# shayneobrien/generative-models

Measured on NVIDIA H100. Metric: train_step_images_per_sec, higher is better.
Workload: dtype bf16

## Files before the change

generative-models_b200/gm_b200/csrc/engine.cu:

```cuda
#include <cstdarg>
#include <cstdio>
#include <cstring>
#include <map>
#include <string>
#include <vector>

#include "gm_b200.h"
#include "gemm_wgmma.cuh"
#include "kernels.cuh"
#include "conv_ops.cuh"

using namespace gm;

typedef CUresult (*PFN_encodeTiled)(CUtensorMap*, CUtensorMapDataType, cuuint32_t, void*, const cuuint64_t*,
                                    const cuuint64_t*, const cuuint32_t*, const cuuint32_t*, CUtensorMapInterleave,
                                    CUtensorMapSwizzle, CUtensorMapL2promotion, CUtensorMapFloatOOBfill);

struct gm_ctx {
  int device = 0;
  int num_sms = 0;
  PFN_encodeTiled encode = nullptr;
  std::string err;
  long long launches = 0;
  float* scratch = nullptr;
// ... 45 lines not shown
}
static const Sampler kNoSampler = {0u, 1u, 0ull, 0ull, nullptr, 0ull};

static int make_tmap(gm_ctx* c, CUtensorMap* tm, const void* ptr, uint64_t inner, uint64_t outer, uint64_t ld,
                     uint32_t box_inner, uint32_t box_outer, CUtensorMapSwizzle swizzle = CU_TENSOR_MAP_SWIZZLE_128B) {
  if ((reinterpret_cast<uintptr_t>(ptr) & 15) || (ld * 2) % 16 != 0)
    return fail(c, GM_ERR_ARG, "tensor map: pointer/ld must be 16-byte aligned (ptr=%p ld=%llu)", ptr, (unsigned long long)ld);
  cuuint64_t dims[2] = {inner, outer};
  cuuint64_t strides[1] = {ld * 2};
  cuuint32_t box[2] = {box_inner, box_outer};
  cuuint32_t estr[2] = {1, 1};
  CUresult r = c->encode(tm, CU_TENSOR_MAP_DATA_TYPE_BFLOAT16, 2, const_cast<void*>(ptr), dims, strides, box, estr,
                         CU_TENSOR_MAP_INTERLEAVE_NONE, swizzle, CU_TENSOR_MAP_L2_PROMOTION_L2_256B,
                         CU_TENSOR_MAP_FLOAT_OOB_FILL_NONE);
  if (r != CUDA_SUCCESS) return fail(c, GM_ERR_CUDA, "cuTensorMapEncodeTiled failed with %d", int(r));
  return GM_OK;
}

enum PlanKind { PK_NT_208 = 0, PK_NT_64, PK_TN_256, PK_TN_64 };

struct GemmPlan {
  CUtensorMap tmA, tmB;
  CUtensorMap tmA2, tmB2;
  mutable CUtensorMap tmC;
  mutable int tmc_state;
  GemmParams p;
  int kind;
  int grid;
  double flops;
};

static bool g_pdl = true;
static bool g_tma_store = true;
struct ProfAll { const char* name; cudaEvent_t e0, e1; };
static bool g_prof_all = false;
static std::vector<ProfAll> g_prof_all_recs;
template <typename... KArgs, typename... Args>
static cudaError_t launch_pdl(const char* name, void (*kern)(KArgs...), dim3 grid, dim3 block, size_t smem, cudaStream_t s, Args&&... args) {
  struct Scope {
    cudaStream_t s; ProfAll r; bool on;
    Scope(const char* n, cudaStream_t s_) : s(s_), on(g_prof_all) {
      if (on) { r.name = n; cudaEventCreate(&r.e0); cudaEventCreate(&r.e1); cudaEventRecord(r.e0, s); }
    }
    ~Scope() { if (on) { cudaEventRecord(r.e1, s); g_prof_all_recs.push_back(r); } }
  } scope(name, s);
  const bool pdl = g_pdl && strcmp(name, "xhat_kernel") != 0;
  cudaLaunchConfig_t cfg;
  memset(&cfg, 0, sizeof cfg);
  cfg.gridDim = grid;
  cfg.blockDim = block;
  cfg.dynamicSmemBytes = smem;
  cfg.stream = s;
  cudaLaunchAttribute at[1];
  at[0].id = cudaLaunchAttributeProgrammaticStreamSerialization;
  at[0].val.programmaticStreamSerializationAllowed = 1;
  cfg.attrs = at;
  cfg.numAttrs = pdl ? 1 : 0;
  return cudaLaunchKernelEx(&cfg, kern, KArgs(args)...);
}

template <int BN, bool AMN, bool BMN, int EPI = kEpiUniversal, bool SPLIT = false, bool PP = false>
static cudaError_t launch_inst(const GemmPlan& pl, cudaStream_t s) {
  using Cfg = GemmCfg<BN, !AMN, PP>;
  constexpr int CL = kGemmCluster<BN, AMN, BMN>;
  auto kern = gemm_wgmma_kernel<BN, AMN, BMN, EPI, SPLIT, PP>;
  cudaLaunchConfig_t cfg;
  memset(&cfg, 0, sizeof cfg);
  cfg.gridDim = dim3(pl.grid);
  cfg.blockDim = dim3(kGemmThreads);
  cfg.dynamicSmemBytes = Cfg::SMEM_BYTES;
  cfg.stream = s;
  cudaLaunchAttribute at[2];
  int na = 0;
  if (CL > 1) {
    at[na].id = cudaLaunchAttributeClusterDimension;
    at[na].val.clusterDim.x = CL;
    at[na].val.clusterDim.y = 1;
    at[na].val.clusterDim.z = 1;
    ++na;
  }
  static bool configured[64] = {};
  static int max_clusters[64] = {};
  int dev = 0;
  cudaGetDevice(&dev);
  const bool cached = dev >= 0 && dev < 64;
  int mc = cached ? max_clusters[dev] : 0;
  if (!cached || !configured[dev]) {
    cudaError_t e = cudaFuncSetAttribute(kern, cudaFuncAttributeMaxDynamicSharedMemorySize, Cfg::SMEM_BYTES);
    if (e != cudaSuccess) return e;
    if (CL > 1) {
      cfg.gridDim = dim3(CL);
      cfg.attrs = at;
      cfg.numAttrs = na;
      e = cudaOccupancyMaxActiveClusters(&mc, kern, &cfg);
      if (e != cudaSuccess) return e;
      if (mc < 1) return cudaErrorInvalidConfiguration;
    }
    if (cached) { max_clusters[dev] = mc; configured[dev] = true; }
  }
  if (CL > 1) {
    const GemmParams& q = pl.p;
    const int items = cdiv(q.m_tiles, CL) * q.n_tiles * q.splits;
    cfg.gridDim = dim3(CL * (items < mc ? items : mc));
  }
  if (g_pdl) {
    at[na].id = cudaLaunchAttributeProgrammaticStreamSerialization;
    at[na].val.programmaticStreamSerializationAllowed = 1;
    ++na;
  }
  cfg.attrs = at;
  cfg.numAttrs = na;
  GemmParams prm = pl.p;
  prm.tma_store = pl.tmc_state == 1 ? 1 : 0;
  prm.f32_vec = prm.epi == EPI_F32 && !(reinterpret_cast<uintptr_t>(prm.part) & 15) && prm.ldp % 4 == 0 && prm.part_stride % 4 == 0;
  return cudaLaunchKernelEx(&cfg, kern, pl.tmA, pl.tmB, pl.tmC, pl.tmA2, pl.tmB2, prm);
}

template <int BN, bool AMN, bool BMN>
static cudaError_t launch_split(const GemmPlan& pl, cudaStream_t s) {
  return launch_inst<BN, AMN, BMN, kEpiUniversal, true>(pl, s);
}

constexpr int kPingPongMaxKblocks = 7;

static cudaError_t launch_nt208(const GemmPlan& pl, cudaStream_t s) {
  const GemmParams& p = pl.p;
  if (p.epi != EPI_BF16) return launch_inst<208, false, false>(pl, s);
  const bool pp = p.kblocks <= kPingPongMaxKblocks;
#define NT208(S) case S: return launch_inst<208, false, false, S>(pl, s)
#define NT208_PINGPONG(S) case S: return pp ? launch_inst<208, false, false, S, false, true>(pl, s) : launch_inst<208, false, false, S>(pl, s)
  switch (epi_sig(p)) {
    NT208_PINGPONG(epi_sig(ACT_RELU, AUX_NONE, true, DOT_NONE));
    NT208_PINGPONG(epi_sig(ACT_SIGMOID, AUX_NONE, true, DOT_NONE));
    NT208(epi_sig(ACT_RELU, AUX_NONE, true, DOT_W));
    NT208(epi_sig(ACT_RELU, AUX_NONE, true, DOT_W_MASK));
    NT208(epi_sig(ACT_RELU, AUX_NONE, true, DOT_W_PRE));
    NT208(epi_sig(ACT_NONE, AUX_NONE, false, DOT_NONE));
    NT208(epi_sig(ACT_NONE, AUX_NONE, false, DOT_SQ));
// ... 4 lines not shown
    NT208(epi_sig(ACT_SIGMOID, AUX_VAE_OUT, true, DOT_NONE));
    default: return launch_inst<208, false, false>(pl, s);
  }
#undef NT208
#undef NT208_PINGPONG
}

static int launch_plan(gm_ctx* c, const GemmPlan& pl, cudaStream_t s) {
  if (pl.tmc_state == 0) {
    const GemmParams& p = pl.p;
    const bool nt = pl.kind == PK_NT_208 || pl.kind == PK_NT_64;
    pl.tmc_state = 2;
    if (g_tma_store && nt && epi_plain(p.aux_mode, p.dot) && p.nparts == 1 && p.epi == EPI_BF16 && p.out != nullptr && !(reinterpret_cast<uintptr_t>(p.out) & 15) &&
        (p.ldo * 2) % 16 == 0 && p.out_cols > 0) {
      int rc = make_tmap(c, &pl.tmC, p.out, uint64_t(p.out_cols), uint64_t(p.M), uint64_t(p.ldo), kEpiCols, kEpiRows, CU_TENSOR_MAP_SWIZZLE_64B);
      if (rc) return rc;
      pl.tmc_state = 1;
    }
  }
  cudaError_t e;
  gm_ctx::ProfRec rec;
  ProfAll pa;
  if (g_prof_all) {
    static const char* kKind[4] = {"gemm_nt208", "gemm_nt64", "gemm_tn256", "gemm_tn64"};
    static std::map<int, std::string> names;
    const GemmParams& q = pl.p;
    const bool f32 = q.epi == EPI_F32, klong = q.K >= 512, split = q.nparts == 3;
    const int key = epi_sig(q) | (pl.kind | f32 << 2 | klong << 3 | split << 4) << kEpiSigBits;
    auto it = names.find(key);
    if (it == names.end()) {
      char buf[128];
      snprintf(buf, sizeof buf, "%s[act%d aux%d%s%s%s%s%s K%s%s]", kKind[pl.kind], q.act, q.aux_mode, q.bias ? " bias" : "",
               dot_has_w(q.dot) ? " dot" : "", q.dot == DOT_W_PRE ? " pre" : (q.dot == DOT_W_MASK ? " mask" : ""),
               q.dot == DOT_SQ ? " sq" : "", f32 ? " f32" : "", klong ? "long" : "short", split ? " split" : "");
      it = names.emplace(key, buf).first;
    }
    pa.name = it->second.c_str();
    cudaEventCreate(&pa.e0); cudaEventCreate(&pa.e1);
    cudaEventRecord(pa.e0, s);
  }
  if (c->prof) {
    cudaEventCreate(&rec.e0);
    cudaEventCreate(&rec.e1);
    rec.kind = pl.kind;
    rec.flops = pl.flops;
    cudaEventRecord(rec.e0, s);
  }
  if (pl.p.nparts == 3) {
    switch (pl.kind) {
      case PK_NT_208: e = launch_split<208, false, false>(pl, s); break;
      case PK_NT_64: e = launch_split<64, false, false>(pl, s); break;
      case PK_TN_256: e = launch_split<256, true, true>(pl, s); break;
      default: e = launch_split<64, true, true>(pl, s); break;
    }
  } else
  switch (pl.kind) {
    case PK_NT_208: e = launch_nt208(pl, s); break;
    case PK_NT_64: e = launch_inst<64, false, false>(pl, s); break;
    case PK_TN_256: e = launch_inst<256, true, true>(pl, s); break;
    default: e = launch_inst<64, true, true>(pl, s); break;
  }
  c->launches++;
  if (c->prof) {
    cudaEventRecord(rec.e1, s);
    c->prof_recs.push_back(rec);
  }
  if (g_prof_all) { cudaEventRecord(pa.e1, s); g_prof_all_recs.push_back(pa); }
  if (e != cudaSuccess) return fail(c, GM_ERR_CUDA, "GEMM launch failed: %s", cudaGetErrorString(e));
  return GM_OK;
}

static int plan_gemm(gm_ctx* c, GemmPlan* pl, int mode, int M, int N, int K, const void* A, int lda, const void* B,
                     int ldb, int ncover, int max_splits) {
  memset(pl, 0, sizeof *pl);
  if (M <= 0 || N <= 0 || K <= 0) return fail(c, GM_ERR_ARG, "gemm: bad extents %d %d %d", M, N, K);
  int bn, boxn = 0, boxm = BM;
  if (mode == 0) {
    if (ncover <= 64) { pl->kind = PK_NT_64; bn = 64; boxn = 64; }
    else {
      pl->kind = PK_NT_208; bn = 208; boxn = 208 / kGemmCluster<208, false, false>; boxm = kGemmABoxRows<208, false>;
    }
    int rc = make_tmap(c, &pl->tmA, A, K, M, lda, BK, boxm);
    if (rc) return rc;
    rc = make_tmap(c, &pl->tmB, B, K, N, ldb, BK, boxn);
    if (rc) return rc;
  } else {
    if (ncover <= 64) { pl->kind = PK_TN_64; bn = 64; }
    else { pl->kind = PK_TN_256; bn = 256; }
    int rc = make_tmap(c, &pl->tmA, A, M, K, lda, 64, BK);
    if (rc) return rc;
    rc = make_tmap(c, &pl->tmB, B, N, K, ldb, 64, BK);
    if (rc) return rc;
  }
  GemmParams& p = pl->p;
  pl->flops = 2.0 * M * N * K;
  p.M = M; p.N = N; p.K = K;
  p.m_tiles = cdiv(M, BM);
  p.n_tiles = cdiv(ncover, bn);
  p.kblocks = cdiv(K, BK);
  p.nparts = 1; p.kb_part = p.kblocks; p.lo_off = 0;
  pl->tmA2 = pl->tmA; pl->tmB2 = pl->tmB;
  if (c->plan_lo > 0) {
    const __nv_bfloat16* A2 = static_cast<const __nv_bfloat16*>(A) + c->plan_lo;
    const __nv_bfloat16* B2 = static_cast<const __nv_bfloat16*>(B) + c->plan_lo;
    int rc;
    if (mode == 0) {
      if ((rc = make_tmap(c, &pl->tmA2, A2, K, M, lda, BK, boxm))) return rc;
      if ((rc = make_tmap(c, &pl->tmB2, B2, K, N, ldb, BK, boxn))) return rc;
    } else {
      if ((rc = make_tmap(c, &pl->tmA2, A2, M, K, lda, 64, BK))) return rc;
      if ((rc = make_tmap(c, &pl->tmB2, B2, N, K, ldb, 64, BK))) return rc;
    }
    p.nparts = 3; p.kblocks = 3 * p.kb_part; p.lo_off = c->plan_lo;
  }
  const int tiles = p.m_tiles * p.n_tiles;
  const int slots = c->num_sms;
  int splits = 1;
  if (max_splits > 1) {
    splits = slots / tiles;
    if (splits > max_splits) splits = max_splits;
    if (splits > p.kblocks) splits = p.kblocks;
    if (splits < 1) splits = 1;
  }
  p.kb_per_split = cdiv(p.kblocks, splits);
  p.splits = cdiv(p.kblocks, p.kb_per_split);
  const int total = tiles * p.splits;
  pl->grid = total < slots ? total : slots;
  return GM_OK;
}

__global__ void reduce_partials_kernel(const float* __restrict__ part, int nsplit, long long stride, long long rows, int cols,
                                       int ld, float* __restrict__ out) {
  griddep_sync();
  const long long k = blockIdx.x * (long long)blockDim.x + threadIdx.x;
// ... 16 lines not shown
  if (!out) return GM_ERR_ARG;
  *out = nullptr;
  gm_ctx* c = new gm_ctx();
  c->device = device;
  *out = c;
  int n = 0;
  if (cudaGetDeviceCount(&n) != cudaSuccess || n <= 0)
    return fail(c, GM_ERR_CUDA, "no CUDA device visible: this library has no CPU fallback");
  CU_OK(c, cudaSetDevice(device));
  cudaDeviceProp prop;
  CU_OK(c, cudaGetDeviceProperties(&prop, device));
  if (prop.major != 9 || prop.minor != 0)
    return fail(c, GM_ERR_UNSUPPORTED, "device is sm_%d%d; this library is built for sm_90a (H100) only", prop.major, prop.minor);
  c->num_sms = prop.multiProcessorCount;
  void* fn = nullptr;
  cudaDriverEntryPointQueryResult q;
  CU_OK(c, cudaGetDriverEntryPoint("cuTensorMapEncodeTiled", &fn, cudaEnableDefault, &q));
  if (!fn || q != cudaDriverEntryPointSuccess) return fail(c, GM_ERR_CUDA, "cuTensorMapEncodeTiled not available");
  c->encode = reinterpret_cast<PFN_encodeTiled>(fn);
  const char* np = getenv("GM_NO_PDL");
  g_pdl = !(np && np[0] == '1');
  const char* nts = getenv("GM_NO_TMA_STORE");
  g_tma_store = !(nts && nts[0] == '1');
  return GM_OK;
}
extern "C" int gm_ctx_destroy(gm_ctx* c) {
  if (!c) return GM_OK;
  if (c->scratch) cudaFree(c->scratch);
  if (c->red) cudaFree(c->red);
  if (c->loss_zero) cudaFree(c->loss_zero);
  delete c;
  return GM_OK;
}
extern "C" const char* gm_last_error(const gm_ctx* c) { return c ? c->err.c_str() : "null ctx"; }
extern "C" int gm_ctx_num_sms(const gm_ctx* c) { return c ? c->num_sms : 0; }
extern "C" long long gm_launch_count(gm_ctx* c, int reset) {
  if (!c) return 0;
  const long long n = c->launches;
  if (reset) c->launches = 0;
  return n;
}

extern "C" int gm_prof_enable(gm_ctx* c, int on) {
  if (!c) return GM_ERR_ARG;
  c->prof = on == 1;
  g_prof_all = on == 2;
// ... 1208 lines not shown
```

generative-models_b200/gm_b200/csrc/gemm_wgmma.cuh:

```cuda
#pragma once
#include "ptx.cuh"

namespace gm {

constexpr int BM = 128;
constexpr int BK = 64;
constexpr int kMmaK = 16;
constexpr int kProducerThreads = 128;
constexpr int kConsumerWarps = 8;
constexpr int kGemmThreads = kProducerThreads + kConsumerWarps * 32;
constexpr int kBarWg0Issued = 1;
constexpr int kBarWg1Issued = 2;
constexpr int kProducerRegs = 40;
constexpr int kConsumerRegs = 232;
static_assert(kProducerThreads * kProducerRegs + kConsumerWarps * 32 * kConsumerRegs <= 65536, "register file");
constexpr int kSmemBudget = 227 * 1024;

enum : int { EPI_BF16 = 0, EPI_F32 = 1 };
enum : int { ACT_NONE = 0, ACT_RELU = 1, ACT_SIGMOID = 2, ACT_LRELU = 3 };
enum : int { AUX_NONE = 0, AUX_SIGMOID_GRAD = 1, AUX_RELU_MASK = 2, AUX_VAE_OUT = 3, AUX_L1 = 4, AUX_NONZERO_MASK = 5 };
enum : int { DOT_NONE = 0, DOT_W = 1, DOT_SQ = 2, DOT_W_MASK = 3, DOT_W_PRE = 4 };
__host__ __device__ constexpr bool dot_has_w(int dot) { return dot == DOT_W || dot == DOT_W_MASK || dot == DOT_W_PRE; }

constexpr int kEpiUniversal = -1;
// ... 56 lines not shown
struct GemmCfg {
  static constexpr int BN = BN_;
  static constexpr bool PINGPONG = PINGPONG_;
  static_assert(!PINGPONG || (STAGED_EPI && BN == 208), "ping-pong: 128 x 208 K-major kernel only");
  static constexpr int A_ROWS = PINGPONG ? BM / 2 : BM;
  static constexpr int A_BYTES = A_ROWS * BK * 2;
  static constexpr int B_BYTES = BN * BK * 2;
  static constexpr int STAGE_BYTES = A_BYTES + B_BYTES;
  static constexpr int EPI_BYTES = kConsumerWarps * (kEpiScratchBytes + (STAGED_EPI ? kEpiVecBytes : 0));
  static_assert(!STAGED_EPI || (BN + kEpiCols - 1) / kEpiCols <= kEpiVecBlocks, "bias/dot staging too small");
  static constexpr int FIXED_BYTES = 1024 + 512 + EPI_BYTES;
  static constexpr int STAGES_RAW = (kSmemBudget - FIXED_BYTES) / STAGE_BYTES;
  static constexpr int STAGES = STAGES_RAW > 8 ? 8 : STAGES_RAW;
  static constexpr int SMEM_BYTES = STAGES * STAGE_BYTES + FIXED_BYTES;
  static constexpr int BOXN = BN;
  static_assert(BN % 16 == 0 && BN <= 256, "wgmma N constraint (and 16-column epilogue chunks)");
  static_assert(STAGES >= 2, "need a pipeline");
  static_assert(BN < 208 || STAGES >= 4, "the 208- and 256-wide kernels need a 4-stage ring to hide TMA latency");
  static_assert(!PINGPONG || (STAGES == 5 && SMEM_BYTES <= kSmemBudget), "ping-pong ring");
};

template <int BN, bool A_MN, bool B_MN>
constexpr int kGemmCluster = (BN == 208 && !A_MN && !B_MN) ? 2 : 1;

template <int BN, bool A_MN, bool B_MN, int EPI = kEpiUniversal, bool SPLIT = false, bool PINGPONG = false>
__global__ void __launch_bounds__(kGemmThreads, 1)
gemm_wgmma_kernel(const __grid_constant__ CUtensorMap tmA, const __grid_constant__ CUtensorMap tmB,
                  const __grid_constant__ CUtensorMap tmC, const __grid_constant__ CUtensorMap tmA2,
                  const __grid_constant__ CUtensorMap tmB2, const GemmParams p) {
  constexpr bool kUniversal = EPI == kEpiUniversal;
  static_assert(!SPLIT || kUniversal, "split operands: universal epilogue only");
  using Cfg = GemmCfg<BN, !A_MN, PINGPONG>;
  constexpr int STAGES = Cfg::STAGES;
  constexpr int CL = kGemmCluster<BN, A_MN, B_MN>;
  constexpr bool PP = PINGPONG;
  constexpr int A_BOX = kGemmABoxRows<BN, A_MN>;
  static_assert(Cfg::A_ROWS % A_BOX == 0, "A tile in whole boxes");
  static_assert(!B_MN || BN % 64 == 0, "MN-major B needs 64-wide atoms");
  static_assert(CL == 1 || (!B_MN && (BN / CL) % 8 == 0 && (Cfg::B_BYTES / CL) % 1024 == 0), "multicast B share");

  extern __shared__ uint8_t smem_raw[];
  const uint32_t smem_base = (smem_u32(smem_raw) + 1023u) & ~1023u;
  const uint32_t bar_base = smem_base + STAGES * Cfg::STAGE_BYTES;
  auto full_bar = [&](int s) { return bar_base + 8u * s; };
  auto empty_bar = [&](int s) { return bar_base + 8u * (STAGES + s); };
  const uint32_t epi_base = bar_base + 512u;

  const int warp = __shfl_sync(0xffffffffu, int(threadIdx.x >> 5), 0);
  const int lane = threadIdx.x & 31;

  griddep_launch();
  if (warp == 0 && lane == 0) {
    tma_prefetch_desc(&tmA);
    tma_prefetch_desc(&tmB);
    if constexpr (SPLIT) { tma_prefetch_desc(&tmA2); tma_prefetch_desc(&tmB2); }
    if (p.tma_store) tma_prefetch_desc(&tmC);
    for (int s = 0; s < STAGES; ++s) {
      mbar_init(full_bar(s), 1);
      mbar_init(empty_bar(s), CL * (PP ? kConsumerWarps / 2 : kConsumerWarps));
    }
    fence_mbar_init();
  }
  if constexpr (CL > 1) cluster_sync();
  else __syncthreads();
  griddep_wait();

  const int rank = CL > 1 ? int(cluster_ctarank()) : 0;
  const int tiles = (p.m_tiles + CL - 1) / CL * p.n_tiles;
  const int total = tiles * p.splits;
  const int first = blockIdx.x / CL, stride = gridDim.x / CL;
  auto halves_of = [&](int rem) -> int {
    if constexpr (PP) return (rem / p.n_tiles) * CL * BM + Cfg::A_ROWS < p.M ? 2 : 1;
    else return 1;
  };
  auto stage_of = [](uint32_t it) { return int(it % STAGES); };
  auto phase_of = [](uint32_t it) { return (it / STAGES) & 1u; };

  if (warp < kProducerThreads / 32) {
    setmaxnreg_dec<kProducerRegs>();
    if (warp == 0) {
      uint32_t it = 0;
      const bool leader = elect_one();
      for (int item = first; item < total; item += stride) {
        const int split = item / tiles;
        const int rem = item - split * tiles;
        const int m0 = ((rem / p.n_tiles) * CL + rank) * BM;
        const int n0 = (rem % p.n_tiles) * BN;
        const int kb0 = split * p.kb_per_split;
        const int kb1 = min(kb0 + p.kb_per_split, p.kblocks);
        const int nh = halves_of(rem);
        for (int h = 0; h < nh; ++h)
        for (int kb = kb0; kb < kb1; ++kb, ++it) {
          const int stage = stage_of(it);
          mbar_wait(empty_bar(stage), phase_of(it) ^ 1u);
          if (leader) {
            const uint32_t a_dst = smem_base + stage * Cfg::STAGE_BYTES;
            const uint32_t b_dst = a_dst + Cfg::A_BYTES;
            int kk = kb, opart = 0;
            if constexpr (SPLIT) { opart = kb / p.kb_part; kk = kb - opart * p.kb_part; }
            const CUtensorMap* const ta = (SPLIT && opart == 2) ? &tmA2 : &tmA;
            const CUtensorMap* const tb = (SPLIT && opart == 1) ? &tmB2 : &tmB;
            const int k0 = kk * BK;
            mbar_arrive_expect_tx(full_bar(stage), Cfg::STAGE_BYTES);
            if constexpr (!A_MN) {
#pragma unroll
              for (int a = 0; a < Cfg::A_ROWS / A_BOX; ++a)
                tma_load_2d(a_dst + a * (A_BOX * BK * 2), ta, full_bar(stage), k0, m0 + h * Cfg::A_ROWS + a * A_BOX);
            } else {
#pragma unroll
              for (int a = 0; a < BM / 64; ++a)
                tma_load_2d(a_dst + a * (BK * 128), ta, full_bar(stage), m0 + a * 64, k0);
            }
            if constexpr (CL > 1) {
              tma_load_2d_multicast(b_dst + rank * (Cfg::B_BYTES / CL), tb, full_bar(stage), k0, n0 + rank * (BN / CL), (1u << CL) - 1);
            } else if constexpr (!B_MN) {
              tma_load_2d(b_dst, tb, full_bar(stage), k0, n0);
            } else {
#pragma unroll
              for (int b = 0; b < BN / 64; ++b)
                tma_load_2d(b_dst + b * (BK * 128), tb, full_bar(stage), n0 + b * 64, k0);
            }
          }
          __syncwarp();
        }
      }
    }
  } else {
    setmaxnreg_inc<kConsumerRegs>();
    const int cw = warp - kProducerThreads / 32;
    const int wg = cw >> 2;
    const int er = lane & 15;
    const int par = lane >> 4;
    const uint32_t scratch_s = epi_base + uint32_t(cw) * kEpiScratchBytes;
    const uint32_t vec_s = epi_base + kConsumerWarps * kEpiScratchBytes + uint32_t(cw) * kEpiVecBytes;
    const int act = kUniversal ? p.act : epi_act(EPI);
    const int aux_mode = kUniversal ? p.aux_mode : epi_aux(EPI);
    const bool has_bias = kUniversal ? p.bias != nullptr : epi_bias(EPI);
    const int dot_mode = kUniversal ? p.dot : epi_dot(EPI);
    const bool has_dot = dot_has_w(dot_mode);
    const bool store_pre = dot_mode == DOT_W_PRE;
    const bool mask_all = dot_mode == DOT_W_MASK;
    const bool has_sq = dot_mode == DOT_SQ;
    constexpr bool kTmaStore = !A_MN && !SPLIT && (kUniversal ? BN != 208 : epi_plain(epi_aux(EPI), epi_dot(EPI)));
    const bool tma_st = kTmaStore && p.tma_store != 0;
    bool st_pending = false;
    auto stage_acquire = [&]() {
      if (st_pending) {
        if (er == 0) bulk_wait_read();
        __syncwarp();
        st_pending = false;
      }
    };
    constexpr uint32_t A_LBO = A_MN ? BK * 128 : 16, A_KADV = A_MN ? kMmaK * 128 : kMmaK * 2;
    constexpr uint32_t B_LBO = B_MN ? BK * 128 : 16, B_KADV = B_MN ? kMmaK * 128 : kMmaK * 2;
    constexpr uint32_t A_WG_OFF = A_MN ? BK * 128 : 64 * 128;
    constexpr uint32_t DESC_HI = (1024u >> 4) | (1u << 30);
    constexpr int kSteps = (BN + kEpiStep - 1) / kEpiStep;
    float acc[BN / 2];
    auto frag_to_scratch = [&](int s) {
#pragma unroll
      for (int t = 0; t < kSteps; ++t) {
        if (t == s) {
#pragma unroll
          for (int jj = 0; jj < kEpiStep / 8; ++jj) {
            const int j = t * (kEpiStep / 8) + jj;
            if (j < BN / 8) {
#pragma unroll
              for (int h = 0; h < 2; ++h) {
                const int r = (lane >> 2) + 8 * h, c = 8 * jj + 2 * (lane & 3);
                const uint32_t a = scratch_s + uint32_t(r) * (kEpiStep * 4) + ((uint32_t(c >> 2) ^ frag_swz(r)) << 4) + uint32_t(c & 3) * 4;
                asm volatile("st.shared.v2.f32 [%0], {%1, %2};" ::"r"(a), "f"(acc[4 * j + 2 * h]), "f"(acc[4 * j + 2 * h + 1]) : "memory");
              }
            }
          }
        }
      }
    };
    auto scratch_ld16 = [&](int c, uint32_t (&r)[16]) {
#pragma unroll
      for (int i = 0; i < 4; ++i) {
        const uint4 v = lds128(scratch_s + uint32_t(er) * (kEpiStep * 4) + ((uint32_t((c >> 2) + i) ^ frag_swz(er)) << 4));
        r[4 * i] = v.x; r[4 * i + 1] = v.y; r[4 * i + 2] = v.z; r[4 * i + 3] = v.w;
      }
    };
    auto release = [&](int s) {
      __syncwarp();
      if (lane == 0) {
        mbar_arrive(empty_bar(s));
        if constexpr (CL > 1) mbar_arrive_cluster(mapa_shared(empty_bar(s), uint32_t(rank ^ 1)));
      }
    };
    int stage = 0;
    uint32_t phase = 0;
    uint32_t it = 0;
#pragma unroll 1
    for (int item = first; item < total; item += stride) {
      const int split = item / tiles;
      const int rem = item - split * tiles;
      const int n_tile = rem % p.n_tiles;
      const int m0 = ((rem / p.n_tiles) * CL + rank) * BM;
      const int n0 = n_tile * BN;
      const int kb0 = split * p.kb_per_split;
      const int kb1 = min(kb0 + p.kb_per_split, p.kblocks);
      const int nh = halves_of(rem);
      if constexpr (PP) {
        if (wg == 1 || it != 0) named_bar_sync(wg == 1 ? kBarWg0Issued : kBarWg1Issued, kConsumerWarps * 32);
        if (wg == 1 && nh == 1) {
          it += uint32_t(kb1 - kb0);
          if (item + stride < total) named_bar_arrive(kBarWg1Issued, kConsumerWarps * 32);
          continue;
        }
      }
      int prev = -1;
      if constexpr (PP) {
        const uint32_t it0 = it + (wg == 1 ? uint32_t(kb1 - kb0) : 0u);
        stage = stage_of(it0);
        phase = phase_of(it0);
        it += uint32_t(nh * (kb1 - kb0));
      }
#pragma unroll 1
      for (int kb = kb0; kb < kb1; ++kb) {
        mbar_wait(full_bar(stage), phase);
        const uint32_t a_src = smem_base + stage * Cfg::STAGE_BYTES + (PP ? 0u : wg * A_WG_OFF);
        const uint32_t b_src = smem_base + stage * Cfg::STAGE_BYTES + Cfg::A_BYTES;
        const uint32_t a_lo = ((a_src >> 4) & 0x3FFFu) | ((A_LBO >> 4) << 16);
        const uint32_t b_lo = ((b_src >> 4) & 0x3FFFu) | ((B_LBO >> 4) << 16);
        wgmma_pin(acc);
        wgmma_fence();
#pragma unroll
        for (int k = 0; k < BK / kMmaK; ++k) {
          const uint64_t da = (uint64_t(DESC_HI) << 32) | (a_lo + k * (A_KADV >> 4));
          const uint64_t db = (uint64_t(DESC_HI) << 32) | (b_lo + k * (B_KADV >> 4));
          const uint32_t sc = (kb > kb0 || k > 0) ? 1u : 0u;
          if constexpr (BN == 256) wgmma_bf16_n256<A_MN, B_MN>(acc, da, db, sc);
          else if constexpr (BN == 208) wgmma_bf16_n208<A_MN, B_MN>(acc, da, db, sc);
          else wgmma_bf16_n64<A_MN, B_MN>(acc, da, db, sc);
        }
        wgmma_commit();
        wgmma_wait<1>();
        wgmma_pin(acc);
        if (prev >= 0) release(prev);
        prev = stage;
        if (++stage == STAGES) { stage = 0; phase ^= 1u; }
      }
      if constexpr (PP) {
        if (wg == 0 || item + stride < total) named_bar_arrive(wg == 0 ? kBarWg0Issued : kBarWg1Issued, kConsumerWarps * 32);
      }
      wgmma_wait<0>();
      wgmma_pin(acc);
      if (prev >= 0) release(prev);
      const int wrow0 = m0 + wg * 64 + (cw & 3) * 16;
      const int row = wrow0 + er;
      const bool row_ok = row < p.M;
      if (!A_MN && !(kUniversal && p.epi == EPI_F32)) {
        const int lr = lane >> 3, lc = lane & 7;
        constexpr int kBlocks = (BN + kEpiCols - 1) / kEpiCols;
        constexpr bool kAuxAsync = !kUniversal && epi_aux(EPI) != AUX_NONE && epi_dot(EPI) == DOT_NONE && !epi_bias(EPI);
        const uint32_t auxt_s = vec_s;
// ... 21 lines not shown
            const int blk = pass * 4 + (lane >> 3), c4 = (lane & 7) * 4;
            const int c = n0 + blk * kEpiCols + c4;
            uint4 bz = make_uint4(0, 0, 0, 0), wz = bz;
            if (blk < kBlocks && c < p.N) {
              if (has_bias) {
                bz = __ldg(reinterpret_cast<const uint4*>(p.bias + c));
                if (act == ACT_SIGMOID) {
                  bz.x = __float_as_uint(0.5f * __uint_as_float(bz.x)); bz.y = __float_as_uint(0.5f * __uint_as_float(bz.y));
                  bz.z = __float_as_uint(0.5f * __uint_as_float(bz.z)); bz.w = __float_as_uint(0.5f * __uint_as_float(bz.w));
                }
              }
              if (has_dot) wz = __ldg(reinterpret_cast<const uint4*>(p.dot_w + c));
            }
            if (has_bias) sts128(vec_s + (blk * kEpiCols + c4) * 4, bz);
            if (has_dot) sts128(vec_s + kEpiVecBytes / 2 + (blk * kEpiCols + c4) * 4, wz);
          }
          __syncwarp();
        }
        if (aux_mode != AUX_NONE) {
          aux_fetch(0);
          const int nitem = item + stride;
          if (nitem < total) {
            const int nrem = nitem - (nitem / tiles) * tiles;
            const int nm0 = ((nrem / p.n_tiles) * CL + rank) * BM + wg * 64 + (cw & 3) * 16;
            const int nn0 = (nrem % p.n_tiles) * BN;
            for (int t = lane; t < kEpiRows * 4; t += 32) {
              const int r = nm0 + (t >> 2), c = nn0 + (t & 3) * 64;
              if (r < p.M && c < p.out_cols)
                asm volatile("prefetch.global.L2 [%0];" ::"l"(p.aux + size_t(r) * p.ld_aux + c));
            }
          }
        }
        float dot = 0.f;
        float l1_scale = 0.f;
        if (aux_mode == AUX_L1) l1_scale = __ldg(p.row_scale + (row < p.row_split ? 0 : 1));
        if (aux_mode == AUX_SIGMOID_GRAD || aux_mode == AUX_RELU_MASK || aux_mode == AUX_NONZERO_MASK) l1_scale = (p.row_vec != nullptr && row_ok) ? __ldg(p.row_vec + row) : 1.f;
#pragma unroll 1
        for (int s = 0; s < kSteps; ++s) {
          const int cs = s * kEpiStep;
          if (n0 + cs >= p.out_cols) break;
          const int bi = 2 * s + par;
          const int cb = bi * kEpiCols;
          const int col0 = n0 + cb;
          const int nch = (cb >= BN || col0 >= p.out_cols) ? 0 : (BN - cb) >= kEpiCols ? 2 : (BN - cb) / 16;
          const bool last_step = (cs + kEpiStep >= BN) || (n0 + cs + kEpiStep >= p.out_cols);
          const bool step_tma = tma_st && BN - cs >= kEpiStep && wrow0 < p.M;
          stage_acquire();
          frag_to_scratch(s);
// ... 229 lines not shown
```

generative-models_b200/gm_b200/csrc/ptx.cuh:

```cuda
#pragma once
#include <cstdint>
#include <cuda.h>
#include <cuda_bf16.h>
#include <cuda_runtime.h>

namespace gm {

#ifndef GM_WATCHDOG_CYCLES
#define GM_WATCHDOG_CYCLES (4000000000LL)
#endif

__device__ __forceinline__ uint32_t smem_u32(const void* p) {
  return static_cast<uint32_t>(__cvta_generic_to_shared(p));
}

__device__ __forceinline__ bool elect_one() {
  uint32_t pred;
  asm volatile(
      "{\n"
      ".reg .pred p;\n"
      "elect.sync _|p, 0xffffffff;\n"
      "selp.u32 %0, 1, 0, p;\n"
      "}\n"
      : "=r"(pred));
// ... 72 lines not shown
      ::"r"(smem_dst), "l"(reinterpret_cast<uint64_t>(tmap)), "r"(bar), "r"(c0), "r"(c1), "h"(cta_mask)
      : "memory");
}

__device__ __forceinline__ void wgmma_fence() { asm volatile("wgmma.fence.sync.aligned;" ::: "memory"); }
__device__ __forceinline__ void wgmma_commit() { asm volatile("wgmma.commit_group.sync.aligned;" ::: "memory"); }
template <int N>
__device__ __forceinline__ void wgmma_wait() { asm volatile("wgmma.wait_group.sync.aligned %0;" ::"n"(N) : "memory"); }
template <int R>
__device__ __forceinline__ void wgmma_pin(float (&d)[R]) {
#pragma unroll
  for (int i = 0; i < R; ++i) asm volatile("" : "+f"(d[i])::"memory");
}

template <int TA, int TB>
__device__ __forceinline__ void wgmma_bf16_n64(float (&d)[32], uint64_t da, uint64_t db, uint32_t scale_d) {
  asm volatile(
      "{\n"
      ".reg .pred p;\n"
      "setp.ne.b32 p, %34, 0;\n"
      "wgmma.mma_async.sync.aligned.m64n64k16.f32.bf16.bf16 {%0,%1,%2,%3,%4,%5,%6,%7,%8,%9,%10,%11,%12,%13,%14,%15,%16,%17,%18,%19,%20,%21,%22,%23,%24,%25,%26,%27,%28,%29,%30,%31}, %32, %33, p, 1, 1, %35, %36;\n"
      "}\n"
      : "+f"(d[0]), "+f"(d[1]), "+f"(d[2]), "+f"(d[3]), "+f"(d[4]), "+f"(d[5]), "+f"(d[6]), "+f"(d[7]), "+f"(d[8]), "+f"(d[9]), "+f"(d[10]), "+f"(d[11]), "+f"(d[12]), "+f"(d[13]), "+f"(d[14]), "+f"(d[15]), "+f"(d[16]), "+f"(d[17]), "+f"(d[18]), "+f"(d[19]), "+f"(d[20]), "+f"(d[21]), "+f"(d[22]), "+f"(d[23]), "+f"(d[24]), "+f"(d[25]), "+f"(d[26]), "+f"(d[27]), "+f"(d[28]), "+f"(d[29]), "+f"(d[30]), "+f"(d[31])
      : "l"(da), "l"(db), "r"(scale_d), "n"(TA), "n"(TB));
}

template <int TA, int TB>
__device__ __forceinline__ void wgmma_bf16_n208(float (&d)[104], uint64_t da, uint64_t db, uint32_t scale_d) {
  asm volatile(
      "{\n"
      ".reg .pred p;\n"
      "setp.ne.b32 p, %106, 0;\n"
      "wgmma.mma_async.sync.aligned.m64n208k16.f32.bf16.bf16 {%0,%1,%2,%3,%4,%5,%6,%7,%8,%9,%10,%11,%12,%13,%14,%15,%16,%17,%18,%19,%20,%21,%22,%23,%24,%25,%26,%27,%28,%29,%30,%31,%32,%33,%34,%35,%36,%37,%38,%39,%40,%41,%42,%43,%44,%45,%46,%47,%48,%49,%50,%51,%52,%53,%54,%55,%56,%57,%58,%59,%60,%61,%62,%63,%64,%65,%66,%67,%68,%69,%70,%71,%72,%73,%74,%75,%76,%77,%78,%79,%80,%81,%82,%83,%84,%85,%86,%87,%88,%89,%90,%91,%92,%93,%94,%95,%96,%97,%98,%99,%100,%101,%102,%103}, %104, %105, p, 1, 1, %107, %108;\n"
      "}\n"
      : "+f"(d[0]), "+f"(d[1]), "+f"(d[2]), "+f"(d[3]), "+f"(d[4]), "+f"(d[5]), "+f"(d[6]), "+f"(d[7]), "+f"(d[8]), "+f"(d[9]), "+f"(d[10]), "+f"(d[11]), "+f"(d[12]), "+f"(d[13]), "+f"(d[14]), "+f"(d[15]), "+f"(d[16]), "+f"(d[17]), "+f"(d[18]), "+f"(d[19]), "+f"(d[20]), "+f"(d[21]), "+f"(d[22]), "+f"(d[23]), "+f"(d[24]), "+f"(d[25]), "+f"(d[26]), "+f"(d[27]), "+f"(d[28]), "+f"(d[29]), "+f"(d[30]), "+f"(d[31]), "+f"(d[32]), "+f"(d[33]), "+f"(d[34]), "+f"(d[35]), "+f"(d[36]), "+f"(d[37]), "+f"(d[38]), "+f"(d[39]), "+f"(d[40]), "+f"(d[41]), "+f"(d[42]), "+f"(d[43]), "+f"(d[44]), "+f"(d[45]), "+f"(d[46]), "+f"(d[47]), "+f"(d[48]), "+f"(d[49]), "+f"(d[50]), "+f"(d[51]), "+f"(d[52]), "+f"(d[53]), "+f"(d[54]), "+f"(d[55]), "+f"(d[56]), "+f"(d[57]), "+f"(d[58]), "+f"(d[59]), "+f"(d[60]), "+f"(d[61]), "+f"(d[62]), "+f"(d[63]), "+f"(d[64]), "+f"(d[65]), "+f"(d[66]), "+f"(d[67]), "+f"(d[68]), "+f"(d[69]), "+f"(d[70]), "+f"(d[71]), "+f"(d[72]), "+f"(d[73]), "+f"(d[74]), "+f"(d[75]), "+f"(d[76]), "+f"(d[77]), "+f"(d[78]), "+f"(d[79]), "+f"(d[80]), "+f"(d[81]), "+f"(d[82]), "+f"(d[83]), "+f"(d[84]), "+f"(d[85]), "+f"(d[86]), "+f"(d[87]), "+f"(d[88]), "+f"(d[89]), "+f"(d[90]), "+f"(d[91]), "+f"(d[92]), "+f"(d[93]), "+f"(d[94]), "+f"(d[95]), "+f"(d[96]), "+f"(d[97]), "+f"(d[98]), "+f"(d[99]), "+f"(d[100]), "+f"(d[101]), "+f"(d[102]), "+f"(d[103])
      : "l"(da), "l"(db), "r"(scale_d), "n"(TA), "n"(TB));
}

template <int TA, int TB>
__device__ __forceinline__ void wgmma_bf16_n256(float (&d)[128], uint64_t da, uint64_t db, uint32_t scale_d) {
  asm volatile(
      "{\n"
      ".reg .pred p;\n"
      "setp.ne.b32 p, %130, 0;\n"
      "wgmma.mma_async.sync.aligned.m64n256k16.f32.bf16.bf16 {%0,%1,%2,%3,%4,%5,%6,%7,%8,%9,%10,%11,%12,%13,%14,%15,%16,%17,%18,%19,%20,%21,%22,%23,%24,%25,%26,%27,%28,%29,%30,%31,%32,%33,%34,%35,%36,%37,%38,%39,%40,%41,%42,%43,%44,%45,%46,%47,%48,%49,%50,%51,%52,%53,%54,%55,%56,%57,%58,%59,%60,%61,%62,%63,%64,%65,%66,%67,%68,%69,%70,%71,%72,%73,%74,%75,%76,%77,%78,%79,%80,%81,%82,%83,%84,%85,%86,%87,%88,%89,%90,%91,%92,%93,%94,%95,%96,%97,%98,%99,%100,%101,%102,%103,%104,%105,%106,%107,%108,%109,%110,%111,%112,%113,%114,%115,%116,%117,%118,%119,%120,%121,%122,%123,%124,%125,%126,%127}, %128, %129, p, 1, 1, %131, %132;\n"
      "}\n"
// ... 88 lines not shown
```

Before: 43.09 million.

## Add 208-wide TN GEMM tiles with paired-CTA A multicast and n16 tail

For TN GEMMs (MN-major operands), the N tile can now be 208 instead of 256 when that covers N with fewer wasted columns and gives an even tile count. The 208 tile is computed as an n192 wgmma plus an n16 wgmma, fed by an extra 16-wide tensor map with 32B swizzle. The two CTAs of a cluster take adjacent N tiles and multicast the shared A tile, so each issues half the A loads. The intent is to cut padded tensor-core work on ragged N and reduce A traffic, at the cost of new descriptor and cluster scheduling code.

```diff
diff --git a/generative-models_b200/gm_b200/csrc/engine.cu b/generative-models_b200/gm_b200/csrc/engine.cu
--- a/generative-models_b200/gm_b200/csrc/engine.cu
+++ b/generative-models_b200/gm_b200/csrc/engine.cu
@@ -91,16 +91,19 @@
 struct GemmPlan {
   CUtensorMap tmA, tmB;
   CUtensorMap tmA2, tmB2;
+  CUtensorMap tmBt, tmB2t;
   mutable CUtensorMap tmC;
   mutable int tmc_state;
   GemmParams p;
   int kind;
+  int bn;
   int grid;
   double flops;
 };
 
 static bool g_pdl = true;
 static bool g_tma_store = true;
+static bool g_tn208 = true;
 struct ProfAll { const char* name; cudaEvent_t e0, e1; };
 static bool g_prof_all = false;
 static std::vector<ProfAll> g_prof_all_recs;
@@ -128,11 +131,11 @@
   return cudaLaunchKernelEx(&cfg, kern, KArgs(args)...);
 }
 
-template <int BN, bool AMN, bool BMN, int EPI = kEpiUniversal, bool SPLIT = false, bool PP = false>
+template <int BN, bool AMN, bool BMN, int EPI = kEpiUniversal, bool SPLIT = false, bool PP = false,
+          int CL = kGemmCluster<BN, AMN, BMN>>
 static cudaError_t launch_inst(const GemmPlan& pl, cudaStream_t s) {
   using Cfg = GemmCfg<BN, !AMN, PP>;
-  constexpr int CL = kGemmCluster<BN, AMN, BMN>;
-  auto kern = gemm_wgmma_kernel<BN, AMN, BMN, EPI, SPLIT, PP>;
+  auto kern = gemm_wgmma_kernel<BN, AMN, BMN, EPI, SPLIT, PP, CL>;
   cudaLaunchConfig_t cfg;
   memset(&cfg, 0, sizeof cfg);
   cfg.gridDim = dim3(pl.grid);
@@ -169,7 +172,7 @@
   }
   if (CL > 1) {
     const GemmParams& q = pl.p;
-    const int items = cdiv(q.m_tiles, CL) * q.n_tiles * q.splits;
+    const int items = (BMN ? q.m_tiles * (q.n_tiles / CL) : cdiv(q.m_tiles, CL) * q.n_tiles) * q.splits;
     cfg.gridDim = dim3(CL * (items < mc ? items : mc));
   }
   if (g_pdl) {
@@ -182,7 +185,13 @@
   GemmParams prm = pl.p;
   prm.tma_store = pl.tmc_state == 1 ? 1 : 0;
   prm.f32_vec = prm.epi == EPI_F32 && !(reinterpret_cast<uintptr_t>(prm.part) & 15) && prm.ldp % 4 == 0 && prm.part_stride % 4 == 0;
-  return cudaLaunchKernelEx(&cfg, kern, pl.tmA, pl.tmB, pl.tmC, pl.tmA2, pl.tmB2, prm);
+  return cudaLaunchKernelEx(&cfg, kern, pl.tmA, pl.tmB, pl.tmC, pl.tmA2, pl.tmB2, pl.tmBt, pl.tmB2t, prm);
+}
+
+template <bool SPLIT>
+static cudaError_t launch_tn(const GemmPlan& pl, cudaStream_t s) {
+  if (pl.bn == 256) return launch_inst<256, true, true, kEpiUniversal, SPLIT>(pl, s);
+  return launch_inst<208, true, true, kEpiUniversal, SPLIT, false, 2>(pl, s);
 }
 
 template <int BN, bool AMN, bool BMN>
@@ -233,15 +242,17 @@
   gm_ctx::ProfRec rec;
   ProfAll pa;
   if (g_prof_all) {
-    static const char* kKind[4] = {"gemm_nt208", "gemm_nt64", "gemm_tn256", "gemm_tn64"};
+    static const char* kKind[4] = {"gemm_nt208", "gemm_nt64", "gemm_tn", "gemm_tn64"};
     static std::map<int, std::string> names;
     const GemmParams& q = pl.p;
     const bool f32 = q.epi == EPI_F32, klong = q.K >= 512, split = q.nparts == 3;
-    const int key = epi_sig(q) | (pl.kind | f32 << 2 | klong << 3 | split << 4) << kEpiSigBits;
+    const int key = epi_sig(q) | (pl.kind | f32 << 2 | klong << 3 | split << 4 | (pl.bn == 208) << 5) << kEpiSigBits;
     auto it = names.find(key);
     if (it == names.end()) {
       char buf[128];
-      snprintf(buf, sizeof buf, "%s[act%d aux%d%s%s%s%s%s K%s%s]", kKind[pl.kind], q.act, q.aux_mode, q.bias ? " bias" : "",
+      char kind[32];
+      snprintf(kind, sizeof kind, pl.kind == PK_TN_256 ? "%s%d" : "%s", kKind[pl.kind], pl.bn);
+      snprintf(buf, sizeof buf, "%s[act%d aux%d%s%s%s%s%s K%s%s]", kind, q.act, q.aux_mode, q.bias ? " bias" : "",
                dot_has_w(q.dot) ? " dot" : "", q.dot == DOT_W_PRE ? " pre" : (q.dot == DOT_W_MASK ? " mask" : ""),
                q.dot == DOT_SQ ? " sq" : "", f32 ? " f32" : "", klong ? "long" : "short", split ? " split" : "");
       it = names.emplace(key, buf).first;
@@ -261,14 +272,14 @@
     switch (pl.kind) {
       case PK_NT_208: e = launch_split<208, false, false>(pl, s); break;
       case PK_NT_64: e = launch_split<64, false, false>(pl, s); break;
-      case PK_TN_256: e = launch_split<256, true, true>(pl, s); break;
+      case PK_TN_256: e = launch_tn<true>(pl, s); break;
       default: e = launch_split<64, true, true>(pl, s); break;
     }
   } else
   switch (pl.kind) {
     case PK_NT_208: e = launch_nt208(pl, s); break;
     case PK_NT_64: e = launch_inst<64, false, false>(pl, s); break;
-    case PK_TN_256: e = launch_inst<256, true, true>(pl, s); break;
+    case PK_TN_256: e = launch_tn<false>(pl, s); break;
     default: e = launch_inst<64, true, true>(pl, s); break;
   }
   c->launches++;
@@ -296,13 +307,16 @@
     rc = make_tmap(c, &pl->tmB, B, K, N, ldb, BK, boxn);
     if (rc) return rc;
   } else {
+    const int n208 = cdiv(ncover, 208);
     if (ncover <= 64) { pl->kind = PK_TN_64; bn = 64; }
-    else { pl->kind = PK_TN_256; bn = 256; }
+    else { pl->kind = PK_TN_256; bn = g_tn208 && n208 % 2 == 0 && n208 <= cdiv(ncover, 256) ? 208 : 256; }
     int rc = make_tmap(c, &pl->tmA, A, M, K, lda, 64, BK);
     if (rc) return rc;
     rc = make_tmap(c, &pl->tmB, B, N, K, ldb, 64, BK);
     if (rc) return rc;
-  }
+    if (bn == 208 && (rc = make_tmap(c, &pl->tmBt, B, N, K, ldb, kTnTail, BK, CU_TENSOR_MAP_SWIZZLE_32B))) return rc;
+  }
+  pl->bn = bn;
   GemmParams& p = pl->p;
   pl->flops = 2.0 * M * N * K;
   p.M = M; p.N = N; p.K = K;
@@ -310,7 +324,7 @@
   p.n_tiles = cdiv(ncover, bn);
   p.kblocks = cdiv(K, BK);
   p.nparts = 1; p.kb_part = p.kblocks; p.lo_off = 0;
-  pl->tmA2 = pl->tmA; pl->tmB2 = pl->tmB;
+  pl->tmA2 = pl->tmA; pl->tmB2 = pl->tmB; pl->tmB2t = pl->tmBt;
   if (c->plan_lo > 0) {
     const __nv_bfloat16* A2 = static_cast<const __nv_bfloat16*>(A) + c->plan_lo;
     const __nv_bfloat16* B2 = static_cast<const __nv_bfloat16*>(B) + c->plan_lo;
@@ -321,6 +335,7 @@
     } else {
       if ((rc = make_tmap(c, &pl->tmA2, A2, M, K, lda, 64, BK))) return rc;
       if ((rc = make_tmap(c, &pl->tmB2, B2, N, K, ldb, 64, BK))) return rc;
+      if (bn == 208 && (rc = make_tmap(c, &pl->tmB2t, B2, N, K, ldb, kTnTail, BK, CU_TENSOR_MAP_SWIZZLE_32B))) return rc;
     }
     p.nparts = 3; p.kblocks = 3 * p.kb_part; p.lo_off = c->plan_lo;
   }
@@ -383,6 +398,8 @@
   g_pdl = !(np && np[0] == '1');
   const char* nts = getenv("GM_NO_TMA_STORE");
   g_tma_store = !(nts && nts[0] == '1');
+  const char* tn = getenv("GM_TN208");
+  g_tn208 = !(tn && tn[0] == '0');
   return GM_OK;
 }
 extern "C" int gm_ctx_destroy(gm_ctx* c) {
diff --git a/generative-models_b200/gm_b200/csrc/gemm_wgmma.cuh b/generative-models_b200/gm_b200/csrc/gemm_wgmma.cuh
--- a/generative-models_b200/gm_b200/csrc/gemm_wgmma.cuh
+++ b/generative-models_b200/gm_b200/csrc/gemm_wgmma.cuh
@@ -102,22 +102,29 @@
 
 template <int BN, bool A_MN, bool B_MN>
 constexpr int kGemmCluster = (BN == 208 && !A_MN && !B_MN) ? 2 : 1;
-
-template <int BN, bool A_MN, bool B_MN, int EPI = kEpiUniversal, bool SPLIT = false, bool PINGPONG = false>
+constexpr int kTnTail = 16;
+
+template <int BN, bool A_MN, bool B_MN, int EPI = kEpiUniversal, bool SPLIT = false, bool PINGPONG = false,
+          int CL = kGemmCluster<BN, A_MN, B_MN>>
 __global__ void __launch_bounds__(kGemmThreads, 1)
 gemm_wgmma_kernel(const __grid_constant__ CUtensorMap tmA, const __grid_constant__ CUtensorMap tmB,
                   const __grid_constant__ CUtensorMap tmC, const __grid_constant__ CUtensorMap tmA2,
-                  const __grid_constant__ CUtensorMap tmB2, const GemmParams p) {
+                  const __grid_constant__ CUtensorMap tmB2, const __grid_constant__ CUtensorMap tmBt,
+                  const __grid_constant__ CUtensorMap tmB2t, const GemmParams p) {
   constexpr bool kUniversal = EPI == kEpiUniversal;
   static_assert(!SPLIT || kUniversal, "split operands: universal epilogue only");
   using Cfg = GemmCfg<BN, !A_MN, PINGPONG>;
   constexpr int STAGES = Cfg::STAGES;
-  constexpr int CL = kGemmCluster<BN, A_MN, B_MN>;
   constexpr bool PP = PINGPONG;
   constexpr int A_BOX = kGemmABoxRows<BN, A_MN>;
   static_assert(Cfg::A_ROWS % A_BOX == 0, "A tile in whole boxes");
-  static_assert(!B_MN || BN % 64 == 0, "MN-major B needs 64-wide atoms");
-  static_assert(CL == 1 || (!B_MN && (BN / CL) % 8 == 0 && (Cfg::B_BYTES / CL) % 1024 == 0), "multicast B share");
+  constexpr bool kTail = B_MN && BN == 208;
+  constexpr int B_BOXES = BN / 64;
+  static_assert(!B_MN || BN % 64 == 0 || kTail, "MN-major B needs 64-wide atoms");
+  static_assert(A_MN == B_MN, "one operand form per kernel");
+  static_assert(CL == 1 || CL == 2, "cluster size");
+  static_assert(CL == 1 || (!B_MN && (BN / CL) % 8 == 0 && (Cfg::B_BYTES / CL) % 1024 == 0) || (B_MN && kTail && BM / CL == 64),
+                "multicast share");
 
   extern __shared__ uint8_t smem_raw[];
   const uint32_t smem_base = (smem_u32(smem_raw) + 1023u) & ~1023u;
@@ -134,6 +141,7 @@
     tma_prefetch_desc(&tmA);
     tma_prefetch_desc(&tmB);
     if constexpr (SPLIT) { tma_prefetch_desc(&tmA2); tma_prefetch_desc(&tmB2); }
+    if constexpr (kTail) { tma_prefetch_desc(&tmBt); if constexpr (SPLIT) tma_prefetch_desc(&tmB2t); }
     if (p.tma_store) tma_prefetch_desc(&tmC);
     for (int s = 0; s < STAGES; ++s) {
       mbar_init(full_bar(s), 1);
@@ -145,8 +153,12 @@
   else __syncthreads();
   griddep_wait();
 
+  constexpr bool kPairN = CL > 1 && B_MN;
   const int rank = CL > 1 ? int(cluster_ctarank()) : 0;
-  const int tiles = (p.m_tiles + CL - 1) / CL * p.n_tiles;
+  const int n_groups = kPairN ? p.n_tiles / CL : p.n_tiles;
+  const int tiles = (kPairN ? p.m_tiles : (p.m_tiles + CL - 1) / CL) * n_groups;
+  auto m0_of = [&](int rem) { return ((rem / n_groups) * (kPairN ? 1 : CL) + (kPairN ? 0 : rank)) * BM; };
+  auto n_tile_of = [&](int rem) { return (rem % n_groups) * (kPairN ? CL : 1) + (kPairN ? rank : 0); };
   const int total = tiles * p.splits;
   const int first = blockIdx.x / CL, stride = gridDim.x / CL;
   auto halves_of = [&](int rem) -> int {
@@ -164,8 +176,8 @@
       for (int item = first; item < total; item += stride) {
         const int split = item / tiles;
         const int rem = item - split * tiles;
-        const int m0 = ((rem / p.n_tiles) * CL + rank) * BM;
-        const int n0 = (rem % p.n_tiles) * BN;
+        const int m0 = m0_of(rem);
+        const int n0 = n_tile_of(rem) * BN;
         const int kb0 = split * p.kb_per_split;
         const int kb1 = min(kb0 + p.kb_per_split, p.kblocks);
         const int nh = halves_of(rem);
@@ -186,19 +198,23 @@
 #pragma unroll
               for (int a = 0; a < Cfg::A_ROWS / A_BOX; ++a)
                 tma_load_2d(a_dst + a * (A_BOX * BK * 2), ta, full_bar(stage), k0, m0 + h * Cfg::A_ROWS + a * A_BOX);
+            } else if constexpr (CL > 1) {
+              tma_load_2d_multicast(a_dst + rank * (BK * 128), ta, full_bar(stage), m0 + rank * 64, k0, (1u << CL) - 1);
             } else {
 #pragma unroll
               for (int a = 0; a < BM / 64; ++a)
                 tma_load_2d(a_dst + a * (BK * 128), ta, full_bar(stage), m0 + a * 64, k0);
             }
-            if constexpr (CL > 1) {
+            if constexpr (CL > 1 && !B_MN) {
               tma_load_2d_multicast(b_dst + rank * (Cfg::B_BYTES / CL), tb, full_bar(stage), k0, n0 + rank * (BN / CL), (1u << CL) - 1);
             } else if constexpr (!B_MN) {
               tma_load_2d(b_dst, tb, full_bar(stage), k0, n0);
             } else {
 #pragma unroll
-              for (int b = 0; b < BN / 64; ++b)
+              for (int b = 0; b < B_BOXES; ++b)
                 tma_load_2d(b_dst + b * (BK * 128), tb, full_bar(stage), n0 + b * 64, k0);
+              if constexpr (kTail)
+                tma_load_2d(b_dst + B_BOXES * (BK * 128), (SPLIT && opart == 1) ? &tmB2t : &tmBt, full_bar(stage), n0 + B_BOXES * 64, k0);
             }
           }
           __syncwarp();
@@ -235,6 +251,8 @@
     constexpr uint32_t B_LBO = B_MN ? BK * 128 : 16, B_KADV = B_MN ? kMmaK * 128 : kMmaK * 2;
     constexpr uint32_t A_WG_OFF = A_MN ? BK * 128 : 64 * 128;
     constexpr uint32_t DESC_HI = (1024u >> 4) | (1u << 30);
+    constexpr uint32_t TAIL_LBO = BK * kTnTail * 2, TAIL_KADV = kMmaK * kTnTail * 2;
+    constexpr uint32_t TAIL_DESC_HI = ((8u * kTnTail * 2) >> 4) | (3u << 30);
     constexpr int kSteps = (BN + kEpiStep - 1) / kEpiStep;
     float acc[BN / 2];
     auto frag_to_scratch = [&](int s) {
@@ -277,8 +295,8 @@
     for (int item = first; item < total; item += stride) {
       const int split = item / tiles;
       const int rem = item - split * tiles;
-      const int n_tile = rem % p.n_tiles;
-      const int m0 = ((rem / p.n_tiles) * CL + rank) * BM;
+      const int n_tile = n_tile_of(rem);
+      const int m0 = m0_of(rem);
       const int n0 = n_tile * BN;
       const int kb0 = split * p.kb_per_split;
       const int kb1 = min(kb0 + p.kb_per_split, p.kblocks);
@@ -305,6 +323,7 @@
         const uint32_t b_src = smem_base + stage * Cfg::STAGE_BYTES + Cfg::A_BYTES;
         const uint32_t a_lo = ((a_src >> 4) & 0x3FFFu) | ((A_LBO >> 4) << 16);
         const uint32_t b_lo = ((b_src >> 4) & 0x3FFFu) | ((B_LBO >> 4) << 16);
+        const uint32_t t_lo = (((b_src + B_BOXES * (BK * 128)) >> 4) & 0x3FFFu) | ((TAIL_LBO >> 4) << 16);
         wgmma_pin(acc);
         wgmma_fence();
 #pragma unroll
@@ -313,7 +332,11 @@
           const uint64_t db = (uint64_t(DESC_HI) << 32) | (b_lo + k * (B_KADV >> 4));
           const uint32_t sc = (kb > kb0 || k > 0) ? 1u : 0u;
           if constexpr (BN == 256) wgmma_bf16_n256<A_MN, B_MN>(acc, da, db, sc);
-          else if constexpr (BN == 208) wgmma_bf16_n208<A_MN, B_MN>(acc, da, db, sc);
+          else if constexpr (kTail) {
+            const uint64_t dt = (uint64_t(TAIL_DESC_HI) << 32) | (t_lo + k * (TAIL_KADV >> 4));
+            wgmma_bf16_n192<A_MN, B_MN, 0>(acc, da, db, sc);
+            wgmma_bf16_n16<A_MN, B_MN, 96>(acc, da, dt, sc);
+          } else if constexpr (BN == 208) wgmma_bf16_n208<A_MN, B_MN>(acc, da, db, sc);
           else wgmma_bf16_n64<A_MN, B_MN>(acc, da, db, sc);
         }
         wgmma_commit();
@@ -381,8 +404,8 @@
           const int nitem = item + stride;
           if (nitem < total) {
             const int nrem = nitem - (nitem / tiles) * tiles;
-            const int nm0 = ((nrem / p.n_tiles) * CL + rank) * BM + wg * 64 + (cw & 3) * 16;
-            const int nn0 = (nrem % p.n_tiles) * BN;
+            const int nm0 = m0_of(nrem) + wg * 64 + (cw & 3) * 16;
+            const int nn0 = n_tile_of(nrem) * BN;
             for (int t = lane; t < kEpiRows * 4; t += 32) {
               const int r = nm0 + (t >> 2), c = nn0 + (t & 3) * 64;
               if (r < p.M && c < p.out_cols)
diff --git a/generative-models_b200/gm_b200/csrc/ptx.cuh b/generative-models_b200/gm_b200/csrc/ptx.cuh
--- a/generative-models_b200/gm_b200/csrc/ptx.cuh
+++ b/generative-models_b200/gm_b200/csrc/ptx.cuh
@@ -118,6 +118,32 @@
       "wgmma.mma_async.sync.aligned.m64n64k16.f32.bf16.bf16 {%0,%1,%2,%3,%4,%5,%6,%7,%8,%9,%10,%11,%12,%13,%14,%15,%16,%17,%18,%19,%20,%21,%22,%23,%24,%25,%26,%27,%28,%29,%30,%31}, %32, %33, p, 1, 1, %35, %36;\n"
       "}\n"
       : "+f"(d[0]), "+f"(d[1]), "+f"(d[2]), "+f"(d[3]), "+f"(d[4]), "+f"(d[5]), "+f"(d[6]), "+f"(d[7]), "+f"(d[8]), "+f"(d[9]), "+f"(d[10]), "+f"(d[11]), "+f"(d[12]), "+f"(d[13]), "+f"(d[14]), "+f"(d[15]), "+f"(d[16]), "+f"(d[17]), "+f"(d[18]), "+f"(d[19]), "+f"(d[20]), "+f"(d[21]), "+f"(d[22]), "+f"(d[23]), "+f"(d[24]), "+f"(d[25]), "+f"(d[26]), "+f"(d[27]), "+f"(d[28]), "+f"(d[29]), "+f"(d[30]), "+f"(d[31])
+      : "l"(da), "l"(db), "r"(scale_d), "n"(TA), "n"(TB));
+}
+
+template <int TA, int TB, int O, int R>
+__device__ __forceinline__ void wgmma_bf16_n16(float (&d)[R], uint64_t da, uint64_t db, uint32_t scale_d) {
+  static_assert(O + 8 <= R, "accumulator range");
+  asm volatile(
+      "{\n"
+      ".reg .pred p;\n"
+      "setp.ne.b32 p, %10, 0;\n"
+      "wgmma.mma_async.sync.aligned.m64n16k16.f32.bf16.bf16 {%0,%1,%2,%3,%4,%5,%6,%7}, %8, %9, p, 1, 1, %11, %12;\n"
+      "}\n"
+      : "+f"(d[O + 0]), "+f"(d[O + 1]), "+f"(d[O + 2]), "+f"(d[O + 3]), "+f"(d[O + 4]), "+f"(d[O + 5]), "+f"(d[O + 6]), "+f"(d[O + 7])
+      : "l"(da), "l"(db), "r"(scale_d), "n"(TA), "n"(TB));
+}
+
+template <int TA, int TB, int O, int R>
+__device__ __forceinline__ void wgmma_bf16_n192(float (&d)[R], uint64_t da, uint64_t db, uint32_t scale_d) {
+  static_assert(O + 96 <= R, "accumulator range");
+  asm volatile(
+      "{\n"
+      ".reg .pred p;\n"
+      "setp.ne.b32 p, %98, 0;\n"
+      "wgmma.mma_async.sync.aligned.m64n192k16.f32.bf16.bf16 {%0,%1,%2,%3,%4,%5,%6,%7,%8,%9,%10,%11,%12,%13,%14,%15,%16,%17,%18,%19,%20,%21,%22,%23,%24,%25,%26,%27,%28,%29,%30,%31,%32,%33,%34,%35,%36,%37,%38,%39,%40,%41,%42,%43,%44,%45,%46,%47,%48,%49,%50,%51,%52,%53,%54,%55,%56,%57,%58,%59,%60,%61,%62,%63,%64,%65,%66,%67,%68,%69,%70,%71,%72,%73,%74,%75,%76,%77,%78,%79,%80,%81,%82,%83,%84,%85,%86,%87,%88,%89,%90,%91,%92,%93,%94,%95}, %96, %97, p, 1, 1, %99, %100;\n"
+      "}\n"
+      : "+f"(d[O + 0]), "+f"(d[O + 1]), "+f"(d[O + 2]), "+f"(d[O + 3]), "+f"(d[O + 4]), "+f"(d[O + 5]), "+f"(d[O + 6]), "+f"(d[O + 7]), "+f"(d[O + 8]), "+f"(d[O + 9]), "+f"(d[O + 10]), "+f"(d[O + 11]), "+f"(d[O + 12]), "+f"(d[O + 13]), "+f"(d[O + 14]), "+f"(d[O + 15]), "+f"(d[O + 16]), "+f"(d[O + 17]), "+f"(d[O + 18]), "+f"(d[O + 19]), "+f"(d[O + 20]), "+f"(d[O + 21]), "+f"(d[O + 22]), "+f"(d[O + 23]), "+f"(d[O + 24]), "+f"(d[O + 25]), "+f"(d[O + 26]), "+f"(d[O + 27]), "+f"(d[O + 28]), "+f"(d[O + 29]), "+f"(d[O + 30]), "+f"(d[O + 31]), "+f"(d[O + 32]), "+f"(d[O + 33]), "+f"(d[O + 34]), "+f"(d[O + 35]), "+f"(d[O + 36]), "+f"(d[O + 37]), "+f"(d[O + 38]), "+f"(d[O + 39]), "+f"(d[O + 40]), "+f"(d[O + 41]), "+f"(d[O + 42]), "+f"(d[O + 43]), "+f"(d[O + 44]), "+f"(d[O + 45]), "+f"(d[O + 46]), "+f"(d[O + 47]), "+f"(d[O + 48]), "+f"(d[O + 49]), "+f"(d[O + 50]), "+f"(d[O + 51]), "+f"(d[O + 52]), "+f"(d[O + 53]), "+f"(d[O + 54]), "+f"(d[O + 55]), "+f"(d[O + 56]), "+f"(d[O + 57]), "+f"(d[O + 58]), "+f"(d[O + 59]), "+f"(d[O + 60]), "+f"(d[O + 61]), "+f"(d[O + 62]), "+f"(d[O + 63]), "+f"(d[O + 64]), "+f"(d[O + 65]), "+f"(d[O + 66]), "+f"(d[O + 67]), "+f"(d[O + 68]), "+f"(d[O + 69]), "+f"(d[O + 70]), "+f"(d[O + 71]), "+f"(d[O + 72]), "+f"(d[O + 73]), "+f"(d[O + 74]), "+f"(d[O + 75]), "+f"(d[O + 76]), "+f"(d[O + 77]), "+f"(d[O + 78]), "+f"(d[O + 79]), "+f"(d[O + 80]), "+f"(d[O + 81]), "+f"(d[O + 82]), "+f"(d[O + 83]), "+f"(d[O + 84]), "+f"(d[O + 85]), "+f"(d[O + 86]), "+f"(d[O + 87]), "+f"(d[O + 88]), "+f"(d[O + 89]), "+f"(d[O + 90]), "+f"(d[O + 91]), "+f"(d[O + 92]), "+f"(d[O + 93]), "+f"(d[O + 94]), "+f"(d[O + 95])
       : "l"(da), "l"(db), "r"(scale_d), "n"(TA), "n"(TB));
 }
 
```

New measurement: 46.13 million (median of 6 runs). 1.07x the previous value.
